# bioinfomaticsCSU/deepsignal

Hardware: AMD Instinct MI355X
Metric: CpG sites/sec (batch=512, k=17, sig=360) (higher is better)
Workload: dtype f32; 1 GPU; configs[1]: 1xMI355X, batch=512, random-init CpG model weights, synthetic (17,360) features, fp32; batch=512, kmer_len=17, signal_len=360

## Files before the change

### deepsignal_amd/csrc/ds_engine.cpp

```cpp
#include "../../include/deepsignal_hip.h"
#include "ds_internal.h"
#include "ds_extract.h"
#include "ds_tsv_device.h"
#include "ds_freq.h"
#include "ds_combine.h"
#include "ds_eval.h"
#include "ds_train.h"

#include <algorithm>
#include <cmath>
#include <cstdio>
#include <cstdlib>
#include <cstring>
#include <functional>
#include <map>
#include <string>
#include <vector>

using namespace ds;

namespace {

constexpr int VOCAB = 1024, EMB = 128, HID = 256, NLAYER = 3, NMOD = 11, INC_OUT = 240;
constexpr double BN_EPS = 1e-3;
// ... 33 lines not shown

struct Op {
    OpKind kind;
    KernelClass kernel;
    Operands operands = OPS_FP32;
    int stream;
    int stage;
    bool after_join = false;
    GemmOp gemm{};
    Stem1Op stem1{};
    PoolOp pool{};
    LstmDiagOp lstm{};
    FusedChain fc{};
    int tm = 0;
    Stem23Args sa{};
    HeadFoldedArgs ha{};
    SplitDense sd{};
    LstmXproj xp{};
    double flops = 0;
    hipEvent_t ev0 = nullptr, ev1 = nullptr;
    bool pending = false;
    int run_launches = 0;
    double run_flops = 0;
};

#define DS_KERNEL_NAME(id, name) name,
const char* const kKernelNames[K_COUNT] = {DS_KERNEL_TABLE(DS_KERNEL_NAME)};
#undef DS_KERNEL_NAME
struct KernelStat {
    int64_t launches = 0;
    double total_ms = 0;
    double flops = 0;
};

struct Stage {
    std::string name;
    int stream = 0;
    int launches = 0;
    double flops_per_site = 0;
    double total_ms = 0;
    int64_t calls = 0;
};

#define DS_SPLIT_DENSE_PARTS 4

struct Plan {
    int n = 0;
    std::vector<GemmLaunch> launches;
    GemmLaunch* d_launches = nullptr;
    std::vector<LstmLaunch> lstm_launches;
    std::vector<Op> ops;
    int fc1_parts = 1;
    hipGraphExec_t graph = nullptr;
    int64_t uses = 0, last_use = 0;
};

enum class Ticket { Idle, Forward, Text, Rows };
using dss::Times;

template <class R>
struct TableRuns {
    R* open = nullptr;
    typename R::Tally ended;
    void close()
    {
        if (!open) return;
        ended.add(open->t);
        delete open;
        open = nullptr;
    }
};
struct Block { char* p = nullptr; size_t cap = 0; };

}

struct Slot {
    hipStream_t s0 = nullptr, s1 = nullptr;
    bool owns_s1 = true;
    hipEvent_t ev_fork = nullptr, ev_join = nullptr;
    float* d_in = nullptr;
    int* d_kmer = nullptr;
    float *d_means = nullptr, *d_stds = nullptr, *d_sanums = nullptr, *d_signals = nullptr;
    float *stem_pool = nullptr, *conv2o = nullptr, *conv3o = nullptr;
    float* modout[NMOD] = {nullptr};
    float *pool2 = nullptr, *pool3 = nullptr;
    float *tmpA = nullptr, *tmpS = nullptr, *tmpB = nullptr;
    float* sigfeat = nullptr;
    float* H[2][NLAYER] = {{nullptr}};
    float* Cst[2][NLAYER] = {{nullptr}};
    float* xproj[2] = {nullptr, nullptr};
    float* hlast[2] = {nullptr, nullptr};
    float *fc1o = nullptr, *logits = nullptr, *act = nullptr;
    int* pred = nullptr;
    float* joint = nullptr;
    char* jsplit = nullptr;

    Ticket ticket = Ticket::Idle;
    int submitted_n = 0;
    char* pin_in = nullptr;
    float* pin_act = nullptr;
    int* pin_pred = nullptr;
    Block pin_reads, d_reads;
    Block d_rows, pin_rows;
    int64_t* pin_rowoff = nullptr;
    char* d_rc = nullptr;
    int* pin_rc = nullptr;
// ... 1077 lines not shown
            HIPCHK(h, hipEventRecord(h->cur->ev_join, h->cur->s1));
            HIPCHK(h, hipStreamWaitEvent(h->cur->s0, h->cur->ev_join, 0));
            joined = true;
        }
        if (timed && !op.ev0) {
            HIPCHK(h, hipEventCreate(&op.ev0));
            HIPCHK(h, hipEventCreate(&op.ev1));
        }
        if (timed == 2) {
            HIPCHK(h, hipEventRecord(op.ev0, s));
            op.run_launches = 1; op.run_flops = op.flops;
        } else if (timed == 1) {
            if (head[si] && head[si]->kernel != op.kernel) { int rc = close_run(si); if (rc) return rc; }
            if (!head[si]) {
                head[si] = &op;
                op.run_launches = 0; op.run_flops = 0;
                HIPCHK(h, hipEventRecord(op.ev0, s));
            }
            head[si]->run_launches += 1;
            head[si]->run_flops += op.flops;
        }
        int rc = issue_op(h, plan, op, s);
        if (rc) return rc;
        if (timed == 2) {
            HIPCHK(h, hipEventRecord(op.ev1, s));
            op.pending = true;
        }
    }
    { int rc = close_run(0); if (rc) return rc; rc = close_run(1); if (rc) return rc; }
    if (!joined) {
        HIPCHK(h, hipEventRecord(h->cur->ev_join, h->cur->s1));
        HIPCHK(h, hipStreamWaitEvent(h->cur->s0, h->cur->ev_join, 0));
    }
    return DS_OK;
}

int collect_stage_times(ds_handle* h)
{
    for (Slot& sl : h->slots)
      for (auto& kv : sl.plans)
        for (Op& op : kv.second.ops) {
            if (!op.pending) continue;
            HIPCHK(h, hipEventSynchronize(op.ev1));
            float ms = 0;
            HIPCHK(h, hipEventElapsedTime(&ms, op.ev0, op.ev1));
            h->stages[op.stage].total_ms += ms;
            KernelStat& K = h->kstat[op.kernel];
            K.launches += op.run_launches; K.total_ms += ms; K.flops += op.run_flops;
            op.pending = false;
        }
    return DS_OK;
}

void destroy_plan(ds_handle* h, Plan& p)
{
    if (p.graph) hipGraphExecDestroy(p.graph);
    for (Op& op : p.ops) { if (op.ev0) hipEventDestroy(op.ev0); if (op.ev1) hipEventDestroy(op.ev1); }
    if (p.d_launches) {
        hipFree(p.d_launches);
        auto it = std::find(h->allocs.begin(), h->allocs.end(), (void*)p.d_launches);
        if (it != h->allocs.end()) h->allocs.erase(it);
    }
    p.graph = nullptr; p.d_launches = nullptr; p.ops.clear();
}

constexpr size_t MAX_PLANS_PER_SLOT = 24;

int get_plan(ds_handle* h, int n, Plan** out)
{
    auto& plans = h->cur->plans;
    auto it = plans.find(n);
    if (it == plans.end()) {
        if (plans.size() >= MAX_PLANS_PER_SLOT && !h->profiling) {
            auto victim = plans.end();
            for (auto jt = plans.begin(); jt != plans.end(); ++jt)
                if (jt->first != h->B && (victim == plans.end() || jt->second.last_use < victim->second.last_use)) victim = jt;
            if (victim != plans.end()) {
                HIPCHK(h, hipStreamSynchronize(h->cur->s0));
                HIPCHK(h, hipStreamSynchronize(h->cur->s1));
                destroy_plan(h, victim->second);
                plans.erase(victim);
            }
        }
        Plan p;
        int rc = build_plan(h, n, &p);
        if (rc) return rc;
        it = plans.emplace(n, std::move(p)).first;
        h->stages_done = true;
    }
    it->second.uses += 1;
    it->second.last_use = ++h->plan_tick;
    *out = &it->second;
    return DS_OK;
}

int ensure_graph(ds_handle* h, Plan& plan)
{
    if (plan.graph) return DS_OK;
    hipGraph_t g = nullptr;
    HIPCHK(h, hipStreamBeginCapture(h->cur->s0, hipStreamCaptureModeThreadLocal));
    int rc = enqueue_forward(h, plan, 0);
    hipError_t e = hipStreamEndCapture(h->cur->s0, &g);
    if (rc) { if (g) hipGraphDestroy(g); return rc; }
    if (e != hipSuccess) return fail(h, DS_ERR_HIP, std::string("hipStreamEndCapture: ") + hipGetErrorString(e));
    e = hipGraphInstantiate(&plan.graph, g, nullptr, nullptr, 0);
    hipGraphDestroy(g);
    if (e != hipSuccess) return fail(h, DS_ERR_HIP, std::string("hipGraphInstantiate: ") + hipGetErrorString(e));
    return DS_OK;
}

int run_resident(ds_handle* h, int n)
{
    Plan* plan = nullptr;
    int rc = get_plan(h, n, &plan);
    if (rc) return rc;
    h->cur->last_n = n;
    h->cur->last_fc1_parts = plan->fc1_parts;
    if (h->profiling) {
        rc = collect_stage_times(h);
        if (rc) return rc;
        rc = enqueue_forward(h, *plan, h->profiling);
        if (rc) return rc;
        for (Stage& S : h->stages) S.calls += 1;
        return DS_OK;
    }
    if (h->use_graph && (plan->graph || n == h->B || plan->uses >= 2)) {
        rc = ensure_graph(h, *plan);
        if (rc) return rc;
        HIPCHK(h, hipGraphLaunch(plan->graph, h->cur->s0));
        return DS_OK;
    }
    return enqueue_forward(h, *plan, 0);
}

void prepare_slots(ds_handle* h)
{
    if (!h->use_graph || h->debug || h->serial) return;
    Slot* keep = h->cur;
    const std::string err_before = h->err;
    for (Slot& sl : h->slots) {
        h->cur = &sl;
        Plan* plan = nullptr;
        int rc = get_plan(h, h->B, &plan);
        if (!rc) { plan->uses = 0; rc = ensure_graph(h, *plan); }
        if (rc) {
            fprintf(stderr, "deepsignal_amd: preparing a slot's full-batch plan failed (%s); plans will be built at the first forward\n",
                    h->err.c_str());
            h->err = err_before;
            break;
        }
    }
    h->cur = keep;
}

}

namespace {
template <class F>
auto guarded(ds_handle* h, F&& body) -> decltype(body())
{
    try {
        return body();
    } catch (const std::bad_alloc&) {
        return fail(h, DS_ERR_NOMEM, "out of host memory");
    } catch (const std::exception& e) {
        return fail(h, DS_ERR_INVALID, std::string("internal error: ") + e.what());
    } catch (...) {
        return fail(h, DS_ERR_INVALID, "internal error");
    }
}

template <class R, class Begin>
int open_run(ds_handle* h, TableRuns<R> ds_handle::*runs, const char* call, Begin begin)
{
    if (!h) return DS_ERR_INVALID;
    TableRuns<R>& r = h->*runs;
    if (r.open) return fail(h, DS_ERR_INVALID, std::string(R::ROUTE) + "_" + call + ": a run is open on this handle (" + R::ROUTE + "_end first)");
    r.open = new R();
    std::string err;
    const int rc = begin(*r.open, &err);
    if (rc == DS_OK) return DS_OK;
    delete r.open;
    r.open = nullptr;
    return fail(h, rc, err);
}

template <class R, class Call>
auto in_run(ds_handle* h, TableRuns<R> ds_handle::*runs, const char* call, Call body, const char* opener = "begin")
    -> decltype(body(std::declval<R&>(), (std::string*)nullptr))
{
    if (!h) return DS_ERR_INVALID;
    R* r = (h->*runs).open;
    if (!r) return fail(h, DS_ERR_INVALID, std::string(R::ROUTE) + "_" + call + ": no run is open (" + R::ROUTE + "_" + opener + " first)");
    std::string err;
    const auto rc = body(*r, &err);
    return rc < 0 ? fail(h, (int)rc, err) : rc;
}
// ... 70 lines not shown
    h->lstm_variant = cfg->reserved[3];
    if (cfg->reserved[4] > 0) h->fuse_max_spt = cfg->reserved[4];
    if (cfg->reserved[5] > 0) h->fuse_min_tiles = cfg->reserved[5];
    if (cfg->reserved[6] > 0) h->split_dense_min_n = cfg->reserved[6];
    h->split_dense_narrow = (flags & DS_TUNE_SPLIT_DENSE_NARROW) != 0;
    h->lstm_xproj = h->split && h->is_rnn && !(flags & DS_TUNE_NO_LSTM_XPROJ);
    h->lstm_xproj_all = h->lstm_xproj && (flags & DS_TUNE_LSTM_XPROJ_ALL);
    h->Bp32 = (h->B + 31) / 32 * 32;
    h->JP = (h->J + 31) / 32 * 32;
    h->debug = cfg->reserved[0] != 0;
#define CK(expr) do { hipError_t e_ = (expr); if (e_ != hipSuccess) { fail(nullptr, DS_ERR_HIP, std::string(#expr) + ": " + hipGetErrorString(e_)); ds_destroy(h); return DS_ERR_HIP; } } while (0)
    CK(hipSetDevice(cfg->device));
    CK(configure_fused_kernels());
    CK(configure_split_kernels());
    int nslots = cfg->reserved[1] > 0 ? cfg->reserved[1] : (h->B <= 1024 && !h->bf16 ? 8 : 4);
    nslots = std::max(1, std::min(nslots, 16));
    h->slots.resize(nslots);
    int rc = DS_OK;
    for (Slot& sl : h->slots) {
        h->cur = &sl;
        CK(hipStreamCreateWithFlags(&sl.s0, hipStreamNonBlocking));
        if (h->shared_s1 && &sl != &h->slots[0]) { sl.s1 = h->slots[0].s1; sl.owns_s1 = false; }
        else CK(hipStreamCreateWithFlags(&sl.s1, hipStreamNonBlocking));
        CK(hipEventCreateWithFlags(&sl.ev_fork, hipEventDisableTiming));
        CK(hipEventCreateWithFlags(&sl.ev_join, hipEventDisableTiming));
        if (!rc) rc = alloc_workspace(h);
    }
    h->cur = &h->slots[0];
#undef CK
    if (!rc) {
        if (!rc && (flags & DS_TUNE_DEBUG_STAMPS)) {
            rc = dalloc(h, &h->dbg_stamps, (size_t)NMOD * 1024 * 16);
            if (!rc) hipMemset(h->dbg_stamps, 0, (size_t)NMOD * 1024 * 16 * 8);
            if (!rc) rc = dalloc(h, &h->dbg_lstm, (size_t)32 * 1024 * 8);
            if (!rc) hipMemset(h->dbg_lstm, 0, (size_t)32 * 1024 * 8 * 8);
        }
    }
    if (rc) { g_create_error = h->err; ds_destroy(h); return rc; }
    *out = h;
    return DS_OK;
}

void ds_destroy(ds_handle* h)
{
    if (!h) return;
    hipSetDevice(h->cfg.device);
    for (Slot& sl : h->slots) {
        if (sl.s0) hipStreamSynchronize(sl.s0);
        if (sl.s1) hipStreamSynchronize(sl.s1);
    }
    for (Slot& sl : h->slots) {
        for (auto& kv : sl.plans) {
            if (kv.second.graph) hipGraphExecDestroy(kv.second.graph);
            for (Op& op : kv.second.ops) { if (op.ev0) hipEventDestroy(op.ev0); if (op.ev1) hipEventDestroy(op.ev1); }
        }
        for (void* p : {(void*)sl.pin_in, (void*)sl.pin_act , (void*)sl.pin_rowoff, (void*)sl.pin_rc,
                        (void*)sl.pin_text, (void*)sl.pin_tres, (void*)sl.pin_reads.p, (void*)sl.pin_rows.p})
            if (p) hipHostFree(p);
        for (void* p : {(void*)sl.d_rc, (void*)sl.d_text, (void*)sl.d_tres, (void*)sl.d_reads.p, (void*)sl.d_rows.p})
            if (p) hipFree(p);
        for (hipEvent_t e : sl.tx_ev) if (e) hipEventDestroy(e);
        for (hipEvent_t e : sl.rc_ev) if (e) hipEventDestroy(e);
        if (sl.ev_fork) hipEventDestroy(sl.ev_fork);
        if (sl.ev_join) hipEventDestroy(sl.ev_join);
        if (sl.s0) hipStreamDestroy(sl.s0);
        if (sl.s1 && sl.owns_s1) hipStreamDestroy(sl.s1);
    }
    h->freq.close();
    h->combine.close();
    h->eval.close();
    delete h->train;
    for (void* p : h->allocs) hipFree(p);
    (void)hipGetLastError();
    delete h;
}

static int ds_set_tensor_impl(ds_handle* h, const char* name, const float* data, const int64_t* shape, int32_t ndim)
{
    if (!h || !name || !data || !shape || ndim < 1 || ndim > 8) return fail(h, DS_ERR_INVALID, "ds_set_tensor: bad argument");
    if (h->finalized) return fail(h, DS_ERR_INVALID, "weights already finalized");
    HostTensor t;
    int64_t cnt = 1;
    for (int i = 0; i < ndim; ++i) { t.shape.push_back(shape[i]); cnt *= shape[i]; }
    if (cnt <= 0) return fail(h, DS_ERR_INVALID, "ds_set_tensor: empty tensor");
    t.data.assign(data, data + cnt);
    h->host[name] = std::move(t);
    return DS_OK;
}

static int ds_finalize_weights_impl(ds_handle* h)
{
    if (!h) return DS_ERR_INVALID;
    if (h->finalized) return fail(h, DS_ERR_INVALID, "weights already finalized");
    hipSetDevice(h->cfg.device);
    const size_t allocs_before = h->allocs.size();
    int rc = finalize_weights(h);
    h->weight_allocs.assign(h->allocs.begin() + allocs_before, h->allocs.end());
    if (!rc) prepare_slots(h);
    return rc;
}

static int ds_load_weights_impl(ds_handle* h, const char* path)
{
    if (!h || !path) return fail(h, DS_ERR_INVALID, "ds_load_weights: bad argument");
    FILE* f = fopen(path, "rb");
    if (!f) return fail(h, DS_ERR_IO, std::string("cannot open ") + path);
    auto bad = [&](const char* why) { fclose(f); return fail(h, DS_ERR_IO, std::string(path) + ": " + why); };
    char magic[8];
    uint32_t nt = 0;
    if (fread(magic, 1, 8, f) != 8 || memcmp(magic, "DSAMDW01", 8) != 0) return bad("not a DSAMDW01 file");
    if (fread(&nt, 4, 1, f) != 1 || nt > 100000) return bad("bad tensor count");
    struct Meta { std::string name; std::vector<int64_t> shape; uint64_t off, nbytes; };
    std::vector<Meta> metas(nt);
    if (fseek(f, 0, SEEK_END) != 0) return bad("cannot seek");
    const long fsize_l = ftell(f);
    if (fsize_l < 12 || fseek(f, 12, SEEK_SET) != 0) return bad("cannot seek");
    const uint64_t fsize = (uint64_t)fsize_l;
    for (auto& m : metas) {
        uint16_t ln = 0; uint8_t nd = 0;
        if (fread(&ln, 2, 1, f) != 1) return bad("truncated header");
        m.name.resize(ln);
        if (ln && fread(&m.name[0], 1, ln, f) != ln) return bad("truncated header");
        if (fread(&nd, 1, 1, f) != 1 || nd > 8) return bad("truncated header");
        for (int i = 0; i < nd; ++i) { uint32_t d = 0; if (fread(&d, 4, 1, f) != 1) return bad("truncated header"); m.shape.push_back(d); }
        if (fread(&m.off, 8, 1, f) != 1 || fread(&m.nbytes, 8, 1, f) != 1) return bad("truncated header");
        const uint64_t max_elems = (uint64_t)1 << 32;
        uint64_t cnt = 1;
        for (int64_t d : m.shape) {
            if (d <= 0 || (uint64_t)d > max_elems / cnt) return bad("bad tensor shape");
            cnt *= (uint64_t)d;
        }
        if (m.nbytes != cnt * 4) return bad("tensor byte count does not match its shape");
        if (m.off > fsize || m.nbytes > fsize - m.off) return bad("tensor payload lies outside the file");
    }
    for (auto& m : metas) {
        HostTensor t;
        t.shape = m.shape;
        t.data.resize(m.nbytes / 4);
        if (fseek(f, (long)m.off, SEEK_SET) != 0 || fread(t.data.data(), 1, m.nbytes, f) != m.nbytes) return bad("truncated payload");
        h->host[m.name] = std::move(t);
    }
    fclose(f);
    return ds_finalize_weights(h);
}

static int ds_forward_device_impl(ds_handle* h, int32_t n, const int32_t* d_kmer, const float* d_means, const float* d_stds,
                      const float* d_sanums, const float* d_signals, float* d_act, int32_t* d_pred)
{
    if (!h) return DS_ERR_INVALID;
    if (!h->finalized) return fail(h, DS_ERR_INVALID, "weights not loaded");
    if (n < 0 || n > h->B) return fail(h, DS_ERR_INVALID, "n exceeds max_batch");
    if (h->rc_fine)
        return fail(h, DS_ERR_UNSUPPORTED, "ds_forward_device is not available on a handle with a recheck attached (ds_set_recheck)");
    if (n == 0) return DS_OK;
    if (!d_kmer || !d_means || !d_stds || !d_sanums || !d_signals || !d_act || !d_pred)
        return fail(h, DS_ERR_INVALID, "null buffer");
    HIPCHK(h, hipSetDevice(h->cfg.device));
    h->cur = &h->slots[h->profiling ? 0 : (h->next_slot++ % h->slots.size())];
    HIPCHK(h, launch_gather_inputs(d_kmer, d_means, d_stds, d_sanums, d_signals, h->cur->d_in, n, h->T, h->S, h->B, h->cur->s0));
    int rc = run_resident(h, n);
    if (rc) return rc;
    HIPCHK(h, launch_scatter_outputs(h->cur->act, h->cur->pred, d_act, d_pred, n, h->C, h->cur->s0));
    return DS_OK;
}

int ds_sync(ds_handle* h)
{
    if (!h) return DS_ERR_INVALID;
    for (Slot& sl : h->slots) {
        HIPCHK(h, hipStreamSynchronize(sl.s0));
        HIPCHK(h, hipStreamSynchronize(sl.s1));
    }
    if (h->profiling) return collect_stage_times(h);
    return DS_OK;
}

static int enqueue_recheck(ds_handle* h, Slot& sl, int n);
static int finish_recheck(ds_handle* h, Slot& sl, int n, float* act, int32_t* pred);


static int idle_slot(ds_handle* h, const char* who, Slot** sl)
{
    HIPCHK(h, hipSetDevice(h->cfg.device));
    const int si = (int)(h->next_slot % h->slots.size());
    if (h->slots[si].ticket != Ticket::Idle)
        return fail(h, DS_ERR_INVALID, std::string(who) + ": every slot is in flight; wait the oldest ticket first");
    *sl = &h->slots[si];
    return DS_OK;
}

static void hold(ds_handle* h, Slot& sl, Ticket kind, int n, int32_t* ticket)
{
    sl.ticket = kind;
    sl.submitted_n = n;
    *ticket = (int32_t)(&sl - h->slots.data());
}

static void release(Slot& sl) { sl.ticket = Ticket::Idle; sl.submitted_n = 0; }

static bool tickets_in_flight(const ds_handle* h)
{
    return std::any_of(h->slots.begin(), h->slots.end(), [](const Slot& sl) { return sl.ticket != Ticket::Idle; });
}

static int ticket_slot(ds_handle* h, const char* who, int32_t ticket, Ticket kind, Slot** sl, int* n)
{
    static const char* const carries[] = {"nothing", "forward", "text rows", "rows"};
    if (ticket < 0 || ticket >= (int)h->slots.size() || h->slots[ticket].ticket != kind)
        return fail(h, DS_ERR_INVALID, std::string(who) + ": no " + carries[(int)kind] + " in flight for this ticket");
    HIPCHK(h, hipSetDevice(h->cfg.device));
    *sl = &h->slots[ticket];
    *n = (*sl)->submitted_n;
    return DS_OK;
}

static int stage_host_inputs(ds_handle* h, Slot& sl, int nparts, const int32_t* counts, const int32_t* const* kmer, const float* const* means,
                             const float* const* stds, const float* const* sanums, const float* const* signals)
{
    const InLayout L = in_layout(h);
    if (!sl.pin_in) HIPCHK(h, hipHostMalloc((void**)&sl.pin_in, L.total, hipHostMallocDefault));
    char* dev = reinterpret_cast<char*>(sl.d_in);
    size_t n = 0;
    for (int i = 0; i < nparts; ++i) {
        const size_t c = (size_t)counts[i];
        if (!c) continue;
        const void* src[5] = {kmer[i], means[i], stds[i], sanums[i], signals[i]};
        for (int k = 0; k < 5; ++k) memcpy(sl.pin_in + L.at[k] + n * L.row[k], src[k], c * L.row[k]);
        n += c;
    }
    if (n == (size_t)h->B) {
        HIPCHK(h, hipMemcpyAsync(dev, sl.pin_in, L.total, hipMemcpyHostToDevice, sl.s0));
        return DS_OK;
    }
    for (int k = 0; k < 5; ++k)
        HIPCHK(h, hipMemcpyAsync(dev + L.at[k], sl.pin_in + L.at[k], n * L.row[k], hipMemcpyHostToDevice, sl.s0));
    return DS_OK;
}

static int enqueue_forward_on(ds_handle* h, Slot& sl, int n)
{
    if (!sl.pin_act) {
        HIPCHK(h, hipHostMalloc((void**)&sl.pin_act, ((size_t)h->B * h->C + h->B) * 4, hipHostMallocDefault));
        sl.pin_pred = reinterpret_cast<int*>(sl.pin_act + (size_t)h->B * h->C);
    }
    h->cur = &sl;
    int rc = run_resident(h, n);
    return rc ? rc : enqueue_recheck(h, sl, n);
}

static int enqueue_results(ds_handle* h, Slot& sl, int n)
{
    HIPCHK(h, hipMemcpyAsync(sl.pin_act, sl.act, ((size_t)h->B * h->C + (size_t)n) * 4, hipMemcpyDeviceToHost, sl.s0));
    return DS_OK;
}

static int enqueue_forward_and_results(ds_handle* h, Slot& sl, int n)
{
    int rc = enqueue_forward_on(h, sl, n);
    return rc ? rc : enqueue_results(h, sl, n);
}

static int submit_forward(ds_handle* h, Slot& sl, int n, int32_t* ticket)
{
    h->next_slot++;
    int rc = enqueue_forward_and_results(h, sl, n);
    if (!rc) hold(h, sl, Ticket::Forward, n, ticket);
    return rc;
}

static int take_results(ds_handle* h, Slot& sl, int n, float* act, int32_t* pred)
{
    HIPCHK(h, hipStreamSynchronize(sl.s0));
    memcpy(act, sl.pin_act, (size_t)n * h->C * 4);
    memcpy(pred, sl.pin_pred, (size_t)n * 4);
    release(sl);
    return finish_recheck(h, sl, n, act, pred);
}

static int inputs_to_host(ds_handle* h, Slot& sl, const char* who, size_t n, void* const (&dst)[5])
{
    const InLayout L = in_layout(h);
    const char* in = reinterpret_cast<const char*>(sl.d_in);
    hipError_t e = hipSuccess;
    for (int k = 0; k < 5 && e == hipSuccess; ++k)
        if (dst[k]) e = hipMemcpyAsync(dst[k], in + L.at[k], n * L.row[k], hipMemcpyDeviceToHost, sl.s0);
    if (e == hipSuccess) e = hipStreamSynchronize(sl.s0);
    if (e == hipSuccess) return DS_OK;
    (void)hipGetLastError();
    return fail(h, DS_ERR_HIP, std::string(who) + ": " + hipGetErrorString(e));
}

static int ds_forward_impl(ds_handle* h, int32_t n, const int32_t* kmer, const float* means, const float* stds, const float* sanums,
               const float* signals, float* act, int32_t* pred)
{
    if (!h) return DS_ERR_INVALID;
    if (!h->finalized) return fail(h, DS_ERR_INVALID, "weights not loaded");
    if (n < 0) return fail(h, DS_ERR_INVALID, "negative n");
    if (n == 0) return DS_OK;
    if (!kmer || !means || !stds || !sanums || !signals || !act || !pred) return fail(h, DS_ERR_INVALID, "null buffer");
    HIPCHK(h, hipSetDevice(h->cfg.device));
    if (!h->profiling) {
        if (tickets_in_flight(h)) return fail(h, DS_ERR_INVALID, "ds_forward: ds_submit tickets are still in flight");
        const int nslots = (int)h->slots.size();
        std::vector<int32_t> tickets;
        size_t tail = 0;
        int off_wait = 0, rc = DS_OK;
        for (int off = 0; off < n && !rc; off += h->B) {
            const int m = std::min(h->B, n - off);
            if ((int)(tickets.size() - tail) == nslots) {
                const int mw = std::min(h->B, n - off_wait);
                rc = ds_wait(h, tickets[tail++], act + (size_t)off_wait * h->C, pred + off_wait);
                if (rc) break;
                off_wait += mw;
            }
            int32_t t = -1;
            rc = ds_submit(h, m, kmer + (size_t)off * h->T, means + (size_t)off * h->T, stds + (size_t)off * h->T,
                           sanums + (size_t)off * h->T, signals + (size_t)off * h->S, &t);
            if (!rc) tickets.push_back(t);
        }
        while (tail < tickets.size() && !rc) {
            const int mw = std::min(h->B, n - off_wait);
            rc = ds_wait(h, tickets[tail++], act + (size_t)off_wait * h->C, pred + off_wait);
            off_wait += mw;
        }
        if (rc) {
            const std::string msg = h->err;
            for (Slot& sl : h->slots) {
                if (sl.s0) hipStreamSynchronize(sl.s0);
                if (sl.s1) hipStreamSynchronize(sl.s1);
                release(sl);
                sl.rc_selected = false;
            }
            h->err = msg;
        }
        return rc;
    }
    const InLayout L = in_layout(h);
    Slot& sl = h->slots[0];
    for (int off = 0; off < n; off += h->B) {
        const int m = std::min(h->B, n - off);
        h->cur = &sl;
        const char* src[5] = {(const char*)kmer, (const char*)means, (const char*)stds, (const char*)sanums, (const char*)signals};
        for (int k = 0; k < 5; ++k)
            HIPCHK(h, hipMemcpyAsync(reinterpret_cast<char*>(sl.d_in) + L.at[k], src[k] + (size_t)off * L.row[k], (size_t)m * L.row[k],
                                     hipMemcpyHostToDevice, sl.s0));
        int rc = run_resident(h, m);
        if (rc) return rc;
        rc = enqueue_recheck(h, sl, m);
        if (rc) return rc;
        HIPCHK(h, hipMemcpyAsync(act + (size_t)off * h->C, sl.act, (size_t)m * h->C * 4, hipMemcpyDeviceToHost, sl.s0));
        HIPCHK(h, hipMemcpyAsync(pred + off, sl.pred, (size_t)m * 4, hipMemcpyDeviceToHost, sl.s0));
        rc = ds_sync(h);
        if (rc) return rc;
        rc = finish_recheck(h, sl, m, act + (size_t)off * h->C, pred + off);
        if (rc) return rc;
    }
    return DS_OK;
}

struct RcLayout { size_t index, in, act, pred, total, pin_act, pin_pred, pin_total; };
static RcLayout rc_layout(const ds_handle* h)
{
    const size_t B = h->B, C = h->C;
    RcLayout L;
    L.index = 16;
    L.in = L.index + 4 * B;
    L.act = L.in + in_layout(h).total;
    L.pred = L.act + 4 * B * C;
    L.total = L.pred + 4 * B;
    L.pin_act = L.index + 4 * B;
// ... 103 lines not shown
    if (c->T != f->T) return differs("kmer_len", c->T, f->T);
    if (c->S != f->S) return differs("signal_len", c->S, f->S);
    if (c->C != f->C) return differs("class_num", c->C, f->C);
    if (c->is_cnn != f->is_cnn) return differs("is_cnn", c->is_cnn, f->is_cnn);
    if (c->is_rnn != f->is_rnn) return differs("is_rnn", c->is_rnn, f->is_rnn);
    if (c->is_base != f->is_base) return differs("is_base", c->is_base, f->is_base);
    if (c->cfg.device != f->cfg.device) return differs("device", c->cfg.device, f->cfg.device);
    if (c->C != 2)
        return fail(c, DS_ERR_UNSUPPORTED, "ds_set_recheck: class_num " + std::to_string(c->C) + ": the selection rule is defined for two classes");
    if (!c->finalized || !f->finalized) return fail(c, DS_ERR_INVALID, "ds_set_recheck: weights not loaded");
    HIPCHK(c, hipSetDevice(c->cfg.device));
    int rc = alloc_recheck(c);
    if (rc) return rc;
    c->rc_fine = f;
    c->rc_margin = margin;
    c->rc_sites = c->rc_rechecked = c->rc_forwards = 0;
    return DS_OK;
}

int ds_get_recheck_stats(ds_handle* h, int64_t* sites, int64_t* rechecked, int64_t* fine_forwards)
{
    if (!h) return DS_ERR_INVALID;
    if (sites) *sites = h->rc_sites;
    if (rechecked) *rechecked = h->rc_rechecked;
    if (fine_forwards) *fine_forwards = h->rc_forwards;
    return DS_OK;
}

int ds_get_recheck_times(ds_handle* h, int32_t reset, int64_t* launches, double* ms) { return h ? h->rc_t.get(reset, launches, ms) : DS_ERR_INVALID; }

static int ds_recheck_select_impl(ds_handle* h, int32_t n, const float* act, float margin, int32_t* count, int32_t* index)
{
    if (!h) return DS_ERR_INVALID;
    if (!act || !count || !index || n < 1 || n > h->B) return fail(h, DS_ERR_INVALID, "ds_recheck_select: bad argument");
    if (h->C != 2) return fail(h, DS_ERR_UNSUPPORTED, "ds_recheck_select: the selection rule is defined for two classes");
    Slot* idle = nullptr;
    int rc = idle_slot(h, "ds_recheck_select", &idle);
    if (rc) return rc;
    Slot& sl = *idle;
    rc = alloc_recheck(h);
    if (rc) return rc;
    HIPCHK(h, hipMemcpyAsync(sl.act, act, (size_t)n * h->C * 4, hipMemcpyHostToDevice, sl.s0));
    HIPCHK(h, launch_recheck_select(recheck_args(h, sl, n, margin), sl.s0));
    HIPCHK(h, hipMemcpyAsync(sl.pin_rc, sl.d_rc, rc_layout(h).index + 4 * (size_t)n, hipMemcpyDeviceToHost, sl.s0));
    HIPCHK(h, hipStreamSynchronize(sl.s0));
    const int m = sl.pin_rc[0];
    if (m < 0 || m > n) return fail(h, DS_ERR_INVALID, "ds_recheck_select: selection count out of range");
    *count = m;
    memcpy(index, sl.pin_rc + rc_layout(h).index / 4, (size_t)m * 4);
    return DS_OK;
}

static int ds_submit_parts_impl(ds_handle* h, int32_t nparts, const int32_t* counts, const int32_t* const* kmer, const float* const* means,
                                const float* const* stds, const float* const* sanums, const float* const* signals, int32_t* ticket)
{
    if (!h || !ticket) return DS_ERR_INVALID;
    if (!h->finalized) return fail(h, DS_ERR_INVALID, "weights not loaded");
    if (nparts <= 0 || !counts || !kmer || !means || !stds || !sanums || !signals) return fail(h, DS_ERR_INVALID, "null buffer");
    int64_t n64 = 0;
    for (int i = 0; i < nparts; ++i) {
        if (counts[i] < 0) return fail(h, DS_ERR_INVALID, "ds_submit: negative segment length");
        if (counts[i] > 0 && (!kmer[i] || !means[i] || !stds[i] || !sanums[i] || !signals[i])) return fail(h, DS_ERR_INVALID, "null buffer");
        n64 += counts[i];
    }
    if (n64 <= 0 || n64 > h->B) return fail(h, DS_ERR_INVALID, "ds_submit: n must be in [1, max_batch]");
    const int n = (int)n64;
    if (h->profiling) return fail(h, DS_ERR_INVALID, "ds_submit is not available while profiling is on");
    Slot* sl = nullptr;
    int rc = idle_slot(h, "ds_submit", &sl);
    if (!rc) rc = stage_host_inputs(h, *sl, nparts, counts, kmer, means, stds, sanums, signals);
    return rc ? rc : submit_forward(h, *sl, n, ticket);
}

static int ds_submit_impl(ds_handle* h, int32_t n, const int32_t* kmer, const float* means, const float* stds, const float* sanums,
              const float* signals, int32_t* ticket)
{
    if (h && (!kmer || !means || !stds || !sanums || !signals)) return fail(h, DS_ERR_INVALID, "null buffer");
    return ds_submit_parts_impl(h, 1, &n, &kmer, &means, &stds, &sanums, &signals, ticket);
}

static int ds_wait_impl(ds_handle* h, int32_t ticket, float* act, int32_t* pred)
{
    if (!h || !act || !pred) return DS_ERR_INVALID;
    Slot* sl = nullptr;
    int n = 0;
    int rc = ticket_slot(h, "ds_wait", ticket, Ticket::Forward, &sl, &n);
    return rc ? rc : take_results(h, *sl, n, act, pred);
}

static int stage_reads_block(ds_handle* h, Slot& sl, const ds_reads* r, dsx::ExtractPlan* p, size_t extra)
{
    std::string err;
    int rc = dsx::plan(r, h->T, h->S, h->B, p, &err);
    if (rc) return fail(h, rc, err);
    const size_t pin_need = p->image_bytes + extra, dev_need = p->device_bytes + extra;
    rc = grow(h, sl, sl.pin_reads, pin_need, pin_need / 4, true);
    if (!rc) rc = grow(h, sl, sl.d_reads, dev_need, dev_need / 4, false);
    if (rc) return rc;
    dsx::stage(r, *p, sl.pin_reads.p);
    HIPCHK(h, hipMemcpyAsync(sl.d_reads.p, sl.pin_reads.p, p->image_bytes, hipMemcpyHostToDevice, sl.s0));
    return DS_OK;
}

static int stage_reads(ds_handle* h, Slot& sl, const ds_reads* r, dsx::ExtractPlan* p, hipEvent_t* ev)
{
    int rc = stage_reads_block(h, sl, r, p, 0);
    if (rc) return rc;
    const dsx::ExtractArgs a = dsx::device_args(r, *p, sl.d_reads.p);
    HIPCHK(h, dsx::launch(*p, a, sl.d_reads.p, sl.d_kmer, sl.d_means, sl.d_stds, sl.d_sanums, sl.d_signals, sl.s0, ev));
    return DS_OK;
}

static int ds_extract_impl(ds_handle* h, const ds_reads* r, int32_t* kmer, float* means, float* stds, float* sanums, float* signals)
{
    if (!h) return DS_ERR_INVALID;
    if (!kmer || !means || !stds || !sanums || !signals) return fail(h, DS_ERR_INVALID, "null buffer");
    Slot* sl = nullptr;
    int rc = idle_slot(h, "ds_extract", &sl);
    if (rc) return rc;
    CallEvents<3> ev;
    const bool timed = h->profiling != 0;
    if (timed) HIPCHK(h, ev.create());
    dsx::ExtractPlan p;
    rc = stage_reads(h, *sl, r, &p, timed ? ev.ev : nullptr);
    if (!rc) rc = inputs_to_host(h, *sl, "ds_extract", (size_t)p.nsites, {kmer, means, stds, sanums, signals});
    if (!rc && timed) {
        float ms0 = 0, ms1 = 0;
        hipEventElapsedTime(&ms0, ev.ev[0], ev.ev[1]);
        hipEventElapsedTime(&ms1, ev.ev[1], ev.ev[2]);
        h->kstat[K_EXTRACT_STATS].launches += 1; h->kstat[K_EXTRACT_STATS].total_ms += ms0;
        h->kstat[K_EXTRACT_SITES].launches += 1; h->kstat[K_EXTRACT_SITES].total_ms += ms1;
// ... 1002 lines not shown
    if (int rc = train_ready(h, "ds_train_get_mask")) return rc;
    const int sid = dstr::stream_index(stream);
    if (sid < 0 || !out) return fail(h, DS_ERR_INVALID, std::string("ds_train_get_mask: unknown stream ") + (stream ? stream : "(null)"));
    if (h->train->last_n == 0) return fail(h, DS_ERR_INVALID, "ds_train_get_mask: no step has run yet");
    std::string err;
    const int64_t rc = h->train->get_mask(sid, out, cap, &err);
    return rc < 0 ? fail(h, (int)rc, "ds_train_get_mask: " + err) : rc;
}

int ds_train_end(ds_handle* h)
{
    if (!h) return DS_ERR_INVALID;
    hipSetDevice(h->cfg.device);
    delete h->train;
    h->train = nullptr;
    h->training = false;
    return DS_OK;
}

int ds_train_mask_reference(uint64_t seed, int64_t step, const char* stream, int32_t n, int32_t kmer_len, float keep_prob, uint8_t* out)
{
    const int sid = dstr::stream_index(stream);
    if (sid < 0 || n < 0 || kmer_len < 1 || !out || !(keep_prob > 0.f && keep_prob <= 1.f)) return DS_ERR_INVALID;
    dstr::mask_reference(seed, step, sid, n, kmer_len, keep_prob, out);
    return DS_OK;
}

int ds_get_train_times(ds_handle* h, int32_t reset, int64_t* steps, double* ms)
{
    if (!h || !steps || !ms) return DS_ERR_INVALID;
    *steps = h->train ? h->train->steps_timed : 0;
    for (int i = 0; i < dstr::NPHASE; ++i) ms[i] = h->train ? h->train->ms[i] : 0.0;
    if (reset && h->train) { h->train->steps_timed = 0; for (double& v : h->train->ms) v = 0; }
    return DS_OK;
}

int ds_train_begin(ds_handle* h, const ds_train_config* cfg) { return guarded(h, [&] { return ds_train_begin_impl(h, cfg, false); }); }
int ds_train_begin_base(ds_handle* h, const ds_train_config* cfg) { return guarded(h, [&] { return ds_train_begin_impl(h, cfg, true); }); }
int ds_train_step_base(ds_handle* h, int32_t n, const int32_t* kmer, const float* means, const float* stds, const float* sanums, const int32_t* labels, float lr, float* loss, int32_t* pred) { return guarded(h, [&] { return ds_train_step_impl(h, "ds_train_step_base", false, n, kmer, means, stds, sanums, labels, lr, loss, pred, nullptr); }); }
int ds_train_eval(ds_handle* h, int32_t n, const int32_t* kmer, const float* means, const float* stds, const float* sanums, const int32_t* labels, float* loss, int32_t* pred, float* logits) { return guarded(h, [&] { return ds_train_step_impl(h, "ds_train_eval", true, n, kmer, means, stds, sanums, labels, 0.f, loss, pred, logits); }); }
int ds_train_set_tensor(ds_handle* h, const char* name, const float* data, int64_t count) { return guarded(h, [&] { return ds_train_set_tensor_impl(h, name, data, count); }); }
int ds_train_step(ds_handle* h, int32_t n, const float* means, const float* stds, const float* sanums, const int32_t* labels, float lr, float* loss, int32_t* pred) { return guarded(h, [&] { return ds_train_step_impl(h, "ds_train_step", false, n, nullptr, means, stds, sanums, labels, lr, loss, pred, nullptr); }); }
int ds_train_sync_weights(ds_handle* h) { return guarded(h, [&] { return ds_train_sync_weights_impl(h); }); }
int64_t ds_train_get_tensor(ds_handle* h, const char* name, float* out, int64_t cap) { return guarded(h, [&] { return train_get(h, "ds_train_get_tensor", name, out, cap, false); }); }
int64_t ds_train_get_grad(ds_handle* h, const char* name, float* out, int64_t cap) { return guarded(h, [&] { return train_get(h, "ds_train_get_grad", name, out, cap, true); }); }
int64_t ds_train_get_mask(ds_handle* h, const char* stream, uint8_t* out, int64_t cap) { return guarded(h, [&] { return ds_train_get_mask_impl(h, stream, out, cap); }); }

int ds_create(const ds_config* cfg, ds_handle** out) { return guarded(nullptr, [&] { return ds_create_impl(cfg, out); }); }
int ds_set_tensor(ds_handle* h, const char* name, const float* data, const int64_t* shape, int32_t ndim) { return guarded(h, [&] { return ds_set_tensor_impl(h, name, data, shape, ndim); }); }
int ds_finalize_weights(ds_handle* h) { return guarded(h, [&] { return ds_finalize_weights_impl(h); }); }
int ds_load_weights(ds_handle* h, const char* path) { return guarded(h, [&] { return ds_load_weights_impl(h, path); }); }
int ds_forward_device(ds_handle* h, int32_t n, const int32_t* d_kmer, const float* d_means, const float* d_stds, const float* d_sanums, const float* d_signals, float* d_act, int32_t* d_pred) { return guarded(h, [&] { return ds_forward_device_impl(h, n, d_kmer, d_means, d_stds, d_sanums, d_signals, d_act, d_pred); }); }
int ds_forward(ds_handle* h, int32_t n, const int32_t* kmer, const float* means, const float* stds, const float* sanums, const float* signals, float* act, int32_t* pred) { return guarded(h, [&] { return ds_forward_impl(h, n, kmer, means, stds, sanums, signals, act, pred); }); }
int ds_submit(ds_handle* h, int32_t n, const int32_t* kmer, const float* means, const float* stds, const float* sanums, const float* signals, int32_t* ticket) { return guarded(h, [&] { return ds_submit_impl(h, n, kmer, means, stds, sanums, signals, ticket); }); }
int ds_submit_parts(ds_handle* h, int32_t nparts, const int32_t* counts, const int32_t* const* kmer, const float* const* means, const float* const* stds, const float* const* sanums, const float* const* signals, int32_t* ticket) { return guarded(h, [&] { return ds_submit_parts_impl(h, nparts, counts, kmer, means, stds, sanums, signals, ticket); }); }
int ds_wait(ds_handle* h, int32_t ticket, float* act, int32_t* pred) { return guarded(h, [&] { return ds_wait_impl(h, ticket, act, pred); }); }
int ds_extract(ds_handle* h, const ds_reads* reads, int32_t* kmer, float* means, float* stds, float* sanums, float* signals) { return guarded(h, [&] { return ds_extract_impl(h, reads, kmer, means, stds, sanums, signals); }); }
int ds_submit_reads(ds_handle* h, const ds_reads* reads, int32_t* ticket) { return guarded(h, [&] { return ds_submit_reads_impl(h, reads, ticket); }); }
int ds_submit_rows(ds_handle* h, const ds_reads* reads, const char* info, const int64_t* info_off, int32_t label, int32_t* ticket) { return guarded(h, [&] { return ds_submit_rows_impl(h, reads, info, info_off, label, ticket); }); }
int64_t ds_wait_rows(ds_handle* h, int32_t ticket, char* out, int64_t cap, int64_t* row_off) { return guarded(h, [&] { return ds_wait_rows_impl(h, ticket, out, cap, row_off); }); }
int64_t ds_extract_rows(ds_handle* h, const ds_reads* reads, const char* info, const int64_t* info_off, int32_t label, char* out, int64_t cap, int64_t* row_off) { return guarded(h, [&] { return ds_extract_rows_impl(h, reads, info, info_off, label, out, cap, row_off); }); }
int ds_set_recheck(ds_handle* coarse, ds_handle* fine, float margin) { return guarded(coarse, [&] { return ds_set_recheck_impl(coarse, fine, margin); }); }
int ds_recheck_select(ds_handle* h, int32_t n, const float* act, float margin, int32_t* count, int32_t* index) { return guarded(h, [&] { return ds_recheck_select_impl(h, n, act, margin, count, index); }); }
int64_t ds_format_values(ds_handle* h, int64_t n, const double* values, char* out, int64_t cap) { return guarded(h, [&] { return ds_format_values_impl(h, n, values, out, cap); }); }
int ds_freq_begin_stream(ds_handle* h, int64_t initial_slots, int32_t batch_rows, double prob_cf) { return guarded(h, [&] { return ds_freq_begin_stream_impl(h, initial_slots, batch_rows, prob_cf); }); }
int ds_freq_push(ds_handle* h, int32_t nrows, const int32_t* chrom, const int64_t* pos, const float* act, int32_t class_num, const int32_t* pred, int32_t* status, int32_t* opened) { return guarded(h, [&] { return ds_freq_push_impl(h, nrows, chrom, pos, act, class_num, pred, status, opened); }); }
int ds_freq_values(ds_handle* h, int64_t n, const float* act, int32_t class_num, double* p0, double* p1, int32_t* status) { return guarded(h, [&] { return ds_freq_values_impl(h, n, act, class_num, p0, p1, status); }); }
int ds_freq_begin(ds_handle* h, int64_t total_rows, int32_t batch_rows, double prob_cf) { return guarded(h, [&] { return ds_freq_begin_impl(h, total_rows, batch_rows, prob_cf); }); }
int ds_freq_parse(ds_handle* h, const char* text, int32_t nrows, const int64_t* row_begin, const int64_t* row_end, const int32_t* chrom, const uint8_t* flags, int32_t* status) { return guarded(h, [&] { return ds_freq_parse_impl(h, text, nrows, row_begin, row_end, chrom, flags, status); }); }
int ds_freq_accumulate(ds_handle* h, int32_t nover, const int32_t* row, const int32_t* chrom, const int64_t* pos, const double* p0, const double* p1, const int32_t* met) { return guarded(h, [&] { return ds_freq_accumulate_impl(h, nover, row, chrom, pos, p0, p1, met); }); }
int64_t ds_freq_result(ds_handle* h, int64_t cap, int64_t* first_row, int32_t* chrom, int64_t* pos, double* sum0, double* sum1, int32_t* met, int32_t* unmet, int64_t* rows, int64_t* used) { return guarded(h, [&] { return ds_freq_result_impl(h, cap, first_row, chrom, pos, sum0, sum1, met, unmet, rows, used); }); }
int ds_eval_begin(ds_handle* h, int64_t total_rows, int32_t batch_rows, int32_t ncf, const double* cf) { return guarded(h, [&] { return ds_eval_begin_impl(h, total_rows, batch_rows, ncf, cf); }); }
int ds_eval_parse(ds_handle* h, const char* text, int32_t nrows, const int64_t* row_begin, const int64_t* row_end, const uint8_t* flags, int32_t* status) { return guarded(h, [&] { return ds_eval_parse_impl(h, text, nrows, row_begin, row_end, flags, status); }); }
int ds_eval_accumulate(ds_handle* h, const uint8_t* mask, int32_t nover, const int32_t* row, const double* p0, const double* p1, const int32_t* called) { return guarded(h, [&] { return ds_eval_accumulate_impl(h, mask, nover, row, p0, p1, called); }); }
int ds_eval_result(ds_handle* h, int64_t* counts, uint64_t* u2, int64_t* pn, int64_t* nn, int64_t* rows, int64_t* distinct) { return guarded(h, [&] { return ds_eval_result_impl(h, counts, u2, pn, nn, rows, distinct); }); }
int ds_combine_begin(ds_handle* h, int32_t form, int32_t nrec, const int64_t* rec_len, int64_t total_rows, int32_t batch_rows) { return guarded(h, [&] { return ds_combine_begin_impl(h, form, nrec, rec_len, total_rows, batch_rows); }); }
int ds_combine_genome(ds_handle* h, const char* text, int64_t nseg, const int64_t* seg_begin, const int64_t* seg_end, const int64_t* seg_bit, const uint8_t* seg_carry) { return guarded(h, [&] { return ds_combine_genome_impl(h, text, nseg, seg_begin, seg_end, seg_bit, seg_carry); }); }
int ds_combine_bitmap(ds_handle* h, int64_t cap_words, uint32_t* bitmap) { return guarded(h, [&] { return ds_combine_bitmap_impl(h, cap_words, bitmap); }); }
int ds_combine_parse(ds_handle* h, const char* text, int32_t nrows, const int64_t* row_begin, const int64_t* row_end, const int32_t* chrom, const uint8_t* flags, int32_t* status) { return guarded(h, [&] { return ds_combine_parse_impl(h, text, nrows, row_begin, row_end, chrom, flags, status); }); }
int ds_combine_accumulate(ds_handle* h, int32_t nover, const int32_t* row, const int32_t* status, const int32_t* chrom, const int64_t* pos, const int32_t* plus, const double* a, const double* b, const int64_t* met, const int64_t* unmet, const int64_t* cov) { return guarded(h, [&] { return ds_combine_accumulate_impl(h, nover, row, status, chrom, pos, plus, a, b, met, unmet, cov); }); }
int64_t ds_combine_result(ds_handle* h, int64_t cap, int32_t* chrom, int64_t* pos, double* sum0, double* sum1, int64_t* met, int64_t* unmet, int64_t* cov, int64_t* last_plus, int64_t* rows) { return guarded(h, [&] { return ds_combine_result_impl(h, cap, chrom, pos, sum0, sum1, met, unmet, cov, last_plus, rows); }); }
int ds_submit_text(ds_handle* h, const char* text, int32_t nrows, const int64_t* row_begin, const int64_t* row_end, int32_t* ticket) { return guarded(h, [&] { return ds_submit_text_impl(h, text, nrows, row_begin, row_end, ticket); }); }
int ds_wait_text(ds_handle* h, int32_t ticket, float* act, int32_t* pred, int32_t* kmer, int32_t* labels, char* info, int64_t info_cap, int64_t* info_off) { return guarded(h, [&] { return ds_wait_text_impl(h, ticket, act, pred, kmer, labels, info, info_cap, info_off); }); }
int ds_parse_text(ds_handle* h, const char* text, int32_t nrows, const int64_t* row_begin, const int64_t* row_end, int32_t* kmer, float* means, float* stds, float* lens, float* signals, int32_t* labels, int32_t* info_len, int32_t* status) { return guarded(h, [&] { return ds_parse_text_impl(h, text, nrows, row_begin, row_end, kmer, means, stds, lens, signals, labels, info_len, status); }); }
}
```

Measured before the change: 448,500 sites/s.

## Split the forward graph into per-stream part graphs for cross-slot overlap

For models that have both a CNN and an RNN branch, the single captured forward graph is split into three separately captured graphs: the signal branch on s0, the event branch on s1, and a tail after the join. They are launched with explicit fork and join events, so work from different slots can interleave on the streams instead of each slot's monolithic graph serialising. The cost is extra graph launches and event operations per batch, more graph memory, and a risk of wrong ordering if the part split misses a dependency.

```diff
diff --git a/deepsignal_amd/csrc/ds_engine.cpp b/deepsignal_amd/csrc/ds_engine.cpp
--- a/deepsignal_amd/csrc/ds_engine.cpp
+++ b/deepsignal_amd/csrc/ds_engine.cpp
@@ -109,6 +109,8 @@
     std::vector<Op> ops;
     int fc1_parts = 1;
     hipGraphExec_t graph = nullptr;
+    hipGraphExec_t part[3] = {nullptr, nullptr, nullptr};
+    bool parts_captured = false;
     int64_t uses = 0, last_use = 0;
 };
 
@@ -1292,9 +1294,52 @@
     return DS_OK;
 }
 
+enum Part { PART_SIGNAL = 0, PART_EVENT = 1, PART_TAIL = 2 };
+
+Part part_of(const Op& op) { return op.after_join ? PART_TAIL : (op.stream == 0 ? PART_SIGNAL : PART_EVENT); }
+
+hipStream_t part_stream(const ds_handle* h, Part part) { return part == PART_EVENT ? h->cur->s1 : h->cur->s0; }
+
+int ensure_part_graphs(ds_handle* h, Plan& plan)
+{
+    if (plan.parts_captured) return DS_OK;
+    for (Part part : {PART_SIGNAL, PART_EVENT, PART_TAIL}) {
+        if (plan.part[part]) continue;
+        if (std::none_of(plan.ops.begin(), plan.ops.end(), [&](const Op& op) { return part_of(op) == part; })) continue;
+        hipStream_t s = part_stream(h, part);
+        hipGraph_t g = nullptr;
+        HIPCHK(h, hipStreamBeginCapture(s, hipStreamCaptureModeThreadLocal));
+        int rc = DS_OK;
+        for (Op& op : plan.ops)
+            if (!rc && part_of(op) == part) rc = issue_op(h, plan, op, s);
+        hipError_t e = hipStreamEndCapture(s, &g);
+        if (rc) { if (g) hipGraphDestroy(g); return rc; }
+        if (e != hipSuccess) return fail(h, DS_ERR_HIP, std::string("hipStreamEndCapture: ") + hipGetErrorString(e));
+        e = hipGraphInstantiate(&plan.part[part], g, nullptr, nullptr, 0);
+        hipGraphDestroy(g);
+        if (e != hipSuccess) return fail(h, DS_ERR_HIP, std::string("hipGraphInstantiate: ") + hipGetErrorString(e));
+    }
+    plan.parts_captured = true;
+    return DS_OK;
+}
+
+int issue_parts(ds_handle* h, Plan& plan)
+{
+    HIPCHK(h, hipEventRecord(h->cur->ev_fork, h->cur->s0));
+    HIPCHK(h, hipStreamWaitEvent(h->cur->s1, h->cur->ev_fork, 0));
+    for (Part part : {PART_SIGNAL, PART_EVENT})
+        if (plan.part[part]) HIPCHK(h, hipGraphLaunch(plan.part[part], part_stream(h, part)));
+    HIPCHK(h, hipEventRecord(h->cur->ev_join, h->cur->s1));
+    HIPCHK(h, hipStreamWaitEvent(h->cur->s0, h->cur->ev_join, 0));
+    if (plan.part[PART_TAIL]) HIPCHK(h, hipGraphLaunch(plan.part[PART_TAIL], h->cur->s0));
+    return DS_OK;
+}
+
 void destroy_plan(ds_handle* h, Plan& p)
 {
     if (p.graph) hipGraphExecDestroy(p.graph);
+    for (hipGraphExec_t& g : p.part) { if (g) hipGraphExecDestroy(g); g = nullptr; }
+    p.parts_captured = false;
     for (Op& op : p.ops) { if (op.ev0) hipEventDestroy(op.ev0); if (op.ev1) hipEventDestroy(op.ev1); }
     if (p.d_launches) {
         hipFree(p.d_launches);
@@ -1349,7 +1394,12 @@
     return DS_OK;
 }
 
-int run_resident(ds_handle* h, int n)
+bool splits_graphs(const ds_handle* h)
+{
+    return h->is_cnn && h->is_rnn && !h->fold_fc && h->slots.size() > 1 && !h->serial && !h->debug && !h->shared_s1;
+}
+
+int run_resident(ds_handle* h, int n, bool pipelined = false)
 {
     Plan* plan = nullptr;
     int rc = get_plan(h, n, &plan);
@@ -1364,6 +1414,10 @@
         for (Stage& S : h->stages) S.calls += 1;
         return DS_OK;
     }
+    if (h->use_graph && pipelined && splits_graphs(h) && !h->rc_fine && (plan->parts_captured || n == h->B || plan->uses >= 2)) {
+        rc = ensure_part_graphs(h, *plan);
+        return rc ? rc : issue_parts(h, *plan);
+    }
     if (h->use_graph && (plan->graph || n == h->B || plan->uses >= 2)) {
         rc = ensure_graph(h, *plan);
         if (rc) return rc;
@@ -1383,6 +1437,7 @@
         Plan* plan = nullptr;
         int rc = get_plan(h, h->B, &plan);
         if (!rc) { plan->uses = 0; rc = ensure_graph(h, *plan); }
+        if (!rc && splits_graphs(h)) rc = ensure_part_graphs(h, *plan);
         if (rc) {
             fprintf(stderr, "deepsignal_amd: preparing a slot's full-batch plan failed (%s); plans will be built at the first forward\n",
                     h->err.c_str());
@@ -1559,6 +1614,7 @@
     for (Slot& sl : h->slots) {
         for (auto& kv : sl.plans) {
             if (kv.second.graph) hipGraphExecDestroy(kv.second.graph);
+            for (hipGraphExec_t g : kv.second.part) if (g) hipGraphExecDestroy(g);
             for (Op& op : kv.second.ops) { if (op.ev0) hipEventDestroy(op.ev0); if (op.ev1) hipEventDestroy(op.ev1); }
         }
         for (void* p : {(void*)sl.pin_in, (void*)sl.pin_act , (void*)sl.pin_rowoff, (void*)sl.pin_rc,
@@ -1665,7 +1721,7 @@
     HIPCHK(h, hipSetDevice(h->cfg.device));
     h->cur = &h->slots[h->profiling ? 0 : (h->next_slot++ % h->slots.size())];
     HIPCHK(h, launch_gather_inputs(d_kmer, d_means, d_stds, d_sanums, d_signals, h->cur->d_in, n, h->T, h->S, h->B, h->cur->s0));
-    int rc = run_resident(h, n);
+    int rc = run_resident(h, n, true);
     if (rc) return rc;
     HIPCHK(h, launch_scatter_outputs(h->cur->act, h->cur->pred, d_act, d_pred, n, h->C, h->cur->s0));
     return DS_OK;
@@ -1684,6 +1740,8 @@
 
 static int enqueue_recheck(ds_handle* h, Slot& sl, int n);
 static int finish_recheck(ds_handle* h, Slot& sl, int n, float* act, int32_t* pred);
+static int ds_submit_impl(ds_handle* h, int32_t n, const int32_t* kmer, const float* means, const float* stds, const float* sanums,
+                          const float* signals, int32_t* ticket, bool pipelined);
 
 
 static int idle_slot(ds_handle* h, const char* who, Slot** sl)
@@ -1744,14 +1802,14 @@
     return DS_OK;
 }
 
-static int enqueue_forward_on(ds_handle* h, Slot& sl, int n)
+static int enqueue_forward_on(ds_handle* h, Slot& sl, int n, bool pipelined = false)
 {
     if (!sl.pin_act) {
         HIPCHK(h, hipHostMalloc((void**)&sl.pin_act, ((size_t)h->B * h->C + h->B) * 4, hipHostMallocDefault));
         sl.pin_pred = reinterpret_cast<int*>(sl.pin_act + (size_t)h->B * h->C);
     }
     h->cur = &sl;
-    int rc = run_resident(h, n);
+    int rc = run_resident(h, n, pipelined);
     return rc ? rc : enqueue_recheck(h, sl, n);
 }
 
@@ -1761,16 +1819,16 @@
     return DS_OK;
 }
 
-static int enqueue_forward_and_results(ds_handle* h, Slot& sl, int n)
-{
-    int rc = enqueue_forward_on(h, sl, n);
+static int enqueue_forward_and_results(ds_handle* h, Slot& sl, int n, bool pipelined = false)
+{
+    int rc = enqueue_forward_on(h, sl, n, pipelined);
     return rc ? rc : enqueue_results(h, sl, n);
 }
 
-static int submit_forward(ds_handle* h, Slot& sl, int n, int32_t* ticket)
+static int submit_forward(ds_handle* h, Slot& sl, int n, int32_t* ticket, bool pipelined = false)
 {
     h->next_slot++;
-    int rc = enqueue_forward_and_results(h, sl, n);
+    int rc = enqueue_forward_and_results(h, sl, n, pipelined);
     if (!rc) hold(h, sl, Ticket::Forward, n, ticket);
     return rc;
 }
@@ -1821,8 +1879,8 @@
                 off_wait += mw;
             }
             int32_t t = -1;
-            rc = ds_submit(h, m, kmer + (size_t)off * h->T, means + (size_t)off * h->T, stds + (size_t)off * h->T,
-                           sanums + (size_t)off * h->T, signals + (size_t)off * h->S, &t);
+            rc = ds_submit_impl(h, m, kmer + (size_t)off * h->T, means + (size_t)off * h->T, stds + (size_t)off * h->T,
+                                sanums + (size_t)off * h->T, signals + (size_t)off * h->S, &t, n > h->B);
             if (!rc) tickets.push_back(t);
         }
         while (tail < tickets.size() && !rc) {
@@ -2032,7 +2090,8 @@
 }
 
 static int ds_submit_parts_impl(ds_handle* h, int32_t nparts, const int32_t* counts, const int32_t* const* kmer, const float* const* means,
-                                const float* const* stds, const float* const* sanums, const float* const* signals, int32_t* ticket)
+                                const float* const* stds, const float* const* sanums, const float* const* signals, int32_t* ticket,
+                                bool pipelined = true)
 {
     if (!h || !ticket) return DS_ERR_INVALID;
     if (!h->finalized) return fail(h, DS_ERR_INVALID, "weights not loaded");
@@ -2049,14 +2108,14 @@
     Slot* sl = nullptr;
     int rc = idle_slot(h, "ds_submit", &sl);
     if (!rc) rc = stage_host_inputs(h, *sl, nparts, counts, kmer, means, stds, sanums, signals);
-    return rc ? rc : submit_forward(h, *sl, n, ticket);
+    return rc ? rc : submit_forward(h, *sl, n, ticket, pipelined);
 }
 
 static int ds_submit_impl(ds_handle* h, int32_t n, const int32_t* kmer, const float* means, const float* stds, const float* sanums,
-              const float* signals, int32_t* ticket)
+              const float* signals, int32_t* ticket, bool pipelined)
 {
     if (h && (!kmer || !means || !stds || !sanums || !signals)) return fail(h, DS_ERR_INVALID, "null buffer");
-    return ds_submit_parts_impl(h, 1, &n, &kmer, &means, &stds, &sanums, &signals, ticket);
+    return ds_submit_parts_impl(h, 1, &n, &kmer, &means, &stds, &sanums, &signals, ticket, pipelined);
 }
 
 static int ds_wait_impl(ds_handle* h, int32_t ticket, float* act, int32_t* pred)
@@ -3165,7 +3224,7 @@
 int ds_load_weights(ds_handle* h, const char* path) { return guarded(h, [&] { return ds_load_weights_impl(h, path); }); }
 int ds_forward_device(ds_handle* h, int32_t n, const int32_t* d_kmer, const float* d_means, const float* d_stds, const float* d_sanums, const float* d_signals, float* d_act, int32_t* d_pred) { return guarded(h, [&] { return ds_forward_device_impl(h, n, d_kmer, d_means, d_stds, d_sanums, d_signals, d_act, d_pred); }); }
 int ds_forward(ds_handle* h, int32_t n, const int32_t* kmer, const float* means, const float* stds, const float* sanums, const float* signals, float* act, int32_t* pred) { return guarded(h, [&] { return ds_forward_impl(h, n, kmer, means, stds, sanums, signals, act, pred); }); }
-int ds_submit(ds_handle* h, int32_t n, const int32_t* kmer, const float* means, const float* stds, const float* sanums, const float* signals, int32_t* ticket) { return guarded(h, [&] { return ds_submit_impl(h, n, kmer, means, stds, sanums, signals, ticket); }); }
+int ds_submit(ds_handle* h, int32_t n, const int32_t* kmer, const float* means, const float* stds, const float* sanums, const float* signals, int32_t* ticket) { return guarded(h, [&] { return ds_submit_impl(h, n, kmer, means, stds, sanums, signals, ticket, true); }); }
 int ds_submit_parts(ds_handle* h, int32_t nparts, const int32_t* counts, const int32_t* const* kmer, const float* const* means, const float* const* stds, const float* const* sanums, const float* const* signals, int32_t* ticket) { return guarded(h, [&] { return ds_submit_parts_impl(h, nparts, counts, kmer, means, stds, sanums, signals, ticket); }); }
 int ds_wait(ds_handle* h, int32_t ticket, float* act, int32_t* pred) { return guarded(h, [&] { return ds_wait_impl(h, ticket, act, pred); }); }
 int ds_extract(ds_handle* h, const ds_reads* reads, int32_t* kmer, float* means, float* stds, float* sanums, float* signals) { return guarded(h, [&] { return ds_extract_impl(h, reads, kmer, means, stds, sanums, signals); }); }
```

Result: faster. 455,500 sites/s, median of 6 (+1.6%).
